# valerio98-lab/DQL_multirotor_landing

Measured on AMD Instinct MI355X. Metric: env-steps/sec (whole node), higher is better.
Workload: dtype f32

## Files before the change

dql_multirotor_landing_amd/csrc/dql_device.hpp:

```cpp
#pragma once
#define DQL_ASM_PIN(...) asm volatile("" : __VA_ARGS__)
#define DQL_ASM_BLOCK(text) asm volatile(text ::: "memory")
#define DQL_ASM_VMOV(dst, src) asm("v_mov_b32 %0, %1" : "=v"(dst) : "s"(src))
#define DQL_ASM_FMA_LIT(d, x, k, y) asm("v_fmamk_f32 %0, %1, %2, %3" : "=v"(d) : "v"(x), "n"(__builtin_bit_cast(int, k)), "v"(y))
#define DQL_ASM_FMA_V(d, x, k, y) asm("v_fma_f32 %0, %1, %2, %3" : "=v"(d) : "v"(x), "v"(k), "v"(y))
#define DQL_ASM_FMA_S(d, x, k, y) asm("v_fma_f32 %0, %1, %2, %3" : "=v"(d) : "v"(x), "s"(k), "v"(y))
#include <hip/hip_runtime.h>
#include <stdint.h>

#include "../../include/dql.h"

#define DQL_DEV __device__ __forceinline__
#ifdef DQL_MARK
#define DQL_SECTION(name) do { __builtin_amdgcn_sched_barrier(0); asm volatile("; SECTION " name ::: "memory"); __builtin_amdgcn_sched_barrier(0); } while (0)
#else
#define DQL_SECTION(name) do { } while (0)
#endif
#ifdef DQL_WAVE_CLOCK
#define DQL_MARK_T(e, k) do { if ((k) == DQL_WAVE_CLOCK) { asm volatile("s_waitcnt vmcnt(0) lgkmcnt(0)" ::: "memory"); (e).mark = wall_clock64(); } } while (0)
#define DQL_WAVE_BEGIN(t0) const unsigned long long t0 = wall_clock64()
#define DQL_WAVE_END_VAR(t1) unsigned long long t1 = 0
#define DQL_WAVE_STORED(e, t1) ((t1) = (e).mark)
#define DQL_WAVE_END(t0, t1, elog, n, i, tid) do {                                                                                           \
    if (DQL_WAVE_CLOCK == 7) { asm volatile("s_waitcnt vmcnt(0) lgkmcnt(0)" ::: "memory"); t1 = wall_clock64(); }                            \
// ... 174 lines not shown
    const T t2 = z * fma_(w, T(0.28498786688), T(0.66666662693));
    const T Rr = t2 + t1, hfsq = T(0.5) * f * f, dk = (T)k;
    return dk * T(6.93147180369123816490e-01) - ((hfsq - (s * (hfsq + Rr) + dk * T(1.90821492927058770002e-10))) - f);
  }
  const T t1 = w * (T(3.999999999940941908e-01) + w * (T(2.222219843214978396e-01) + w * T(1.531383769920937332e-01)));
  const T t2 = z * (T(6.666666666666735130e-01) + w * (T(2.857142874366239149e-01) + w * (T(1.818357216161805012e-01) +
               w * T(1.479819860511658591e-01))));
  const T Rr = t2 + t1, hfsq = T(0.5) * f * f, dk = (T)k;
  return dk * T(6.93147180369123816490e-01) - ((hfsq - (s * (hfsq + Rr) + dk * T(1.90821492927058770002e-10))) - f);
}

DQL_DEV void philox4x32(uint32_t c0, uint32_t c1, uint32_t c2, uint32_t c3, uint32_t k0, uint32_t k1, uint32_t out[4], const uint32_t* kv = nullptr) {
#pragma unroll
  for (int r = 0; r < 10; ++r) {
    const uint64_t p0 = (uint64_t)0xD2511F53u * c0, p1 = (uint64_t)0xCD9E8D57u * c2;
    const uint32_t h0 = (uint32_t)(p0 >> 32), l0 = (uint32_t)p0, h1 = (uint32_t)(p1 >> 32), l1 = (uint32_t)p1;
    const uint32_t n0 = h1 ^ c1 ^ (kv ? kv[r] : k0), n2 = h0 ^ c3 ^ (kv ? kv[10 + r] : k1);
    c0 = n0; c1 = l1; c2 = n2; c3 = l0;
    k0 += 0x9E3779B9u; k1 += 0xBB67AE85u;
  }
  out[0] = c0; out[1] = c1; out[2] = c2; out[3] = c3;
}
constexpr uint32_t STREAM_ACTION = 0u, STREAM_INIT = 0xFFFFFFFFu, STREAM_NOISE0 = 16u;
template <typename T> DQL_DEV T u24(uint32_t r) { return (T)(r >> 8) * T(5.9604644775390625e-08); }
template <typename T> DQL_DEV T u24p(uint32_t r) { return (T)((r >> 8) + 1u) * T(5.9604644775390625e-08); }
template <typename T> DQL_DEV void box_muller(uint32_t ra, uint32_t rb, T& n0, T& n1) {
  const T rad = sqrt_(T(-2.0) * det_log(u24p<T>(ra)));
  T s, c;
  det_sincos(T(6.28318530717958623200e+00) * u24<T>(rb), s, c);
  n0 = rad * c; n1 = rad * s;
}

#define DQL_CONST_AS __attribute__((address_space(4)))
template <typename T> struct MdpK {
  T p_max, v_max, a_max, theta_max, delta_theta, beta, sigma_a, min_alt;
  T w_p, w_v, w_theta, w_dur, w_fail, w_succ, delta_t, f_ag, timeout_steps;
  T lim_p[5], lim_v[5], lim_a[5], angles[7];
  T inv_p_max, inv_v_max, inv_a_max, inv_theta_max, dtheta_ratio;
  T tan2_mid[3];
  double gamma;
  int working, goal_logic;
  uint32_t quirks;
};
template <typename T> struct SimK {
  T dt, g, inv_m, I[3], inv_I[3], l, h, kf, km, lkf, kmkf, aup, adn, omax, cd, crd;
  T dtm, dtg, dtI[3];
// ... 539 lines not shown
template <typename T> DQL_DEV void platform_rec_begin(const SimK<T>& s, const Env<T>& e, PlatRec<T>& r) {
  det_sincos(e.mp_phase, r.sn, r.cs);
  platform_step_sincos(s, e, r.sd, r.cd);
}
template <typename T> DQL_DEV void platform_update(const SimK<T>& s, Env<T>& e, PlatRec<T>* rec = nullptr, bool first_in_period = true) {
  if (Fast32<T>::on && rec) {
    if (first_in_period) platform_rec_begin(s, e, *rec);
    platform_set(s, e, rec->sn, rec->cs);
    const T sn = rec->sn, cs = rec->cs;
    const T sd = rec->sd, cd = rec->cd;
    rec->sn = fma_(sn, cd, cs * sd);
    rec->cs = fma_(cs, cd, -(sn * sd));
  } else platform_eval(s, e);
  T ph = fma_(e.mp_w, s.mp_dt, e.mp_phase);
  if (ph >= T(6.28318530717958623200e+00)) ph -= T(6.28318530717958623200e+00);
  e.mp_phase = ph;
}
template <typename T> DQL_DEV void manager_states(const T (&R)[9], T cy, T sy, T vz, T& vz_state, T& yw_state) {
  vz_state = vz;
  const T A00 = fma_(cy, R[0], sy * R[3]), A01 = fma_(cy, R[1], sy * R[4]);
  const T A10 = fma_(cy, R[3], -(sy * R[0])), A11 = fma_(cy, R[4], -(sy * R[1]));
  yw_state = det_atan2(fma_(A10, cy, A11 * sy), fma_(A00, cy, A01 * sy));
}
template <typename T>
DQL_DEV void manager_obs(const SimK<T>& s, Env<T>& e, T cy, T sy, long long mgr_index, uint32_t k0, uint32_t k1,
                         uint32_t step_lo, uint32_t step_hi, uint32_t env_id, uint32_t mgr_in_step, bool with_noise = true, PlatRec<T>* rec = nullptr, const uint32_t* kv = nullptr) {
  const T dxw = e.mp_x - e.p[0], dyw = e.mp_y - e.p[1];
  const T dvx = e.mp_u - e.v[0], dvy = e.mp_v - e.v[1];
  const T rpx = fma_(cy, dxw, sy * dyw), rpy = fma_(cy, dyw, -(sy * dxw));
  const T rvx = fma_(cy, dvx, sy * dvy), rvy = fma_(cy, dvy, -(sy * dvx));
  T opx = rpx, opy = rpy, ovx = rvx, ovy = rvy;
  if (with_noise && s.noisy) {
    uint32_t r[4]; T n0, n1, n2, n3;
    philox4x32(step_lo, step_hi, env_id, STREAM_NOISE0 + mgr_in_step, k0, k1, r, kv);
    box_muller(r[0], r[1], n0, n1); box_muller(r[2], r[3], n2, n3);
    opx = fma_(s.noise_p, n0, opx); opy = fma_(s.noise_p, n1, opy); ovx = fma_(s.noise_v, n2, ovx); ovy = fma_(s.noise_v, n3, ovy);
  }
  T ax_ = T(0.0), ay_ = T(0.0);
  if (!(e.flags & FL_ACC_INIT)) {
    e.vf_x = rvx; if (s.two_axis) e.vf_y = rvy; e.flags |= FL_ACC_INIT;
  } else {
    T dt_;
    if (s.quirks & DQL_Q_FROZEN_ACC_REFERENCE) dt_ = (T)mgr_index * s.mgr_dt;
    else dt_ = s.mgr_dt;
    if (dt_ <= T(0.0)) dt_ = T(0.01);
    if (Fast32<T>::on && !(s.quirks & DQL_Q_FROZEN_ACC_REFERENCE)) {
      ax_ = kalman1d(e.kal_x_x, e.kal_x_P, s.kal_q, s.kal_r, (rvx - e.vf_x) * s.inv_mgr_dt, s.kal_pss, s.kal_kss, s.kal_r_zero != 0);
      if (s.two_axis) ay_ = kalman1d(e.kal_y_x, e.kal_y_P, s.kal_q, s.kal_r, (rvy - e.vf_y) * s.inv_mgr_dt, s.kal_pss, s.kal_kss, s.kal_r_zero != 0);
    } else {
      ax_ = kalman1d(e.kal_x_x, e.kal_x_P, s.kal_q, s.kal_r, (rvx - e.vf_x) / dt_, s.kal_pss, s.kal_kss, s.kal_r_zero != 0);
      if (s.two_axis) ay_ = kalman1d(e.kal_y_x, e.kal_y_P, s.kal_q, s.kal_r, (rvy - e.vf_y) / dt_, s.kal_pss, s.kal_kss, s.kal_r_zero != 0);
    }
    if (!(s.quirks & DQL_Q_FROZEN_ACC_REFERENCE)) { e.vf_x = rvx; if (s.two_axis) e.vf_y = rvy; }
  }
  e.obs_px = opx; e.obs_py = opy; e.obs_vx = ovx; e.obs_vy = ovy; e.obs_ax = ax_; e.obs_ay = ay_;
  if (e.flags & FL_CONTACT) e.flags |= FL_OBS_CONTACT; else e.flags &= ~FL_OBS_CONTACT;
  platform_update(s, e, rec, mgr_in_step == 0);
// ... 200 lines not shown
}

DQL_DEV long long fx_round(double x) {
  x = __builtin_fmin(__builtin_fmax(x, -0x1p50), 0x1p50);
  const double t = x + 0x1.8p52;
  return __double_as_longlong(t) - __double_as_longlong(0x1.8p52);
}

struct StepOut {
  long long target_fx;
  long long target_y_fx;
  long long reward_fx;
  int cell, cell_y;
  int decision, done;
  QRow next;
};

struct PeriodCtx {
  uint32_t k0, k1, step_lo, step_hi;
  int prev_idx, prev_idy, action, action_y;
  bool is_reset;
  bool coin, coin_y;
};
template <typename T, typename TabPtr>
DQL_DEV PeriodCtx period_begin(const SimK<T>& s, Env<T>& e, const QRow& qx, TabPtr qa, TabPtr qb, int mode, uint32_t eps_thr, int ext_action, uint64_t seed,
                               uint32_t env_id, long long step_index, const uint32_t* kv = nullptr) {
  PeriodCtx c;
  c.k0 = (uint32_t)seed; c.k1 = (uint32_t)(seed >> 32); c.step_lo = (uint32_t)step_index; c.step_hi = (uint32_t)((uint64_t)step_index >> 32);
  uint32_t r[4];
  philox4x32(c.step_lo, c.step_hi, env_id, STREAM_ACTION, c.k0, c.k1, r, kv);
  c.is_reset = (e.flags & FL_DONE) != 0;
  c.prev_idx = e.idx_x; c.prev_idy = e.idx_y;
  const bool two = s.two_axis != 0;
  int action = 2, action_y = 2;
  uint32_t r2[4] = {0u, 0u, 0u, 0u};
  if (two) philox4x32(c.step_lo, c.step_hi, env_id, STREAM_ACTION + 1u, c.k0, c.k1, r2, kv);
  if (c.is_reset) {
    e.step_count = 0; e.cur_check = 0; e.code = DQL_NON_TERMINAL; e.cum_x = T(0.0); e.cum_y = T(0.0);
    e.pitch_sp = T(0.0); e.roll_sp = T(0.0);
    if (!(s.quirks & DQL_Q_SHAPING_SURVIVES_RESET)) { e.shp_p = T(0.0); e.shp_v = T(0.0); e.shp_a = T(0.0); e.shpy_p = T(0.0); e.shpy_v = T(0.0); e.shpy_a = T(0.0); }
    T x0;
    if (s.working == 0 && !s.init_uniform) { T n0, n1; box_muller(r[2], r[3], n0, n1); x0 = s.init_sigma * n0; }
    else x0 = fma_(T(2.0) * u24<T>(r[2]), s.p_max, -s.p_max);
    e.p[0] = place_axis(s.init_uniform, x0, e.mp_x, s.p_max);
    e.p[1] = T(0.0); e.p[2] = s.z_init;
    if (two) {
      T y0;
      if (s.working == 0 && !s.init_uniform) { T n0, n1; box_muller(r2[2], r2[3], n0, n1); y0 = s.init_sigma * n0; }
      else y0 = fma_(T(2.0) * u24<T>(r2[2]), s.p_max, -s.p_max);
      e.p[1] = place_axis(s.init_uniform, y0, e.mp_y, s.p_max);
    }
    e.v[0] = e.v[1] = e.v[2] = T(0.0); e.w[0] = e.w[1] = e.w[2] = T(0.0);
    e.q[0] = T(1.0); e.q[1] = e.q[2] = e.q[3] = T(0.0);
    e.flags &= ~(FL_DONE | FL_CONTACT | FL_OBS_CONTACT);
    e.flags |= FL_WAS_RESET;
  } else {
    e.flags &= ~FL_WAS_RESET;
    if (mode == MODE_EXTERNAL) { action = ext_action & 3; action_y = two ? (ext_action >> 2) & 3 : 2; }
    else {
      const int greedy = agent_predict(qx);
      const bool explore = (mode == MODE_TRAIN) && ((r[0] >> 8) < eps_thr);
      action = explore ? (int)(((uint64_t)r[1] * 3u) >> 32) : greedy;
      if (two) {
        const int greedy_y = agent_predict(qa, qb, c.prev_idy < 0 ? 0 : c.prev_idy);
        const bool explore_y = (mode == MODE_TRAIN) && ((r2[0] >> 8) < eps_thr);
        action_y = explore_y ? (int)(((uint64_t)r2[1] * 3u) >> 32) : greedy_y;
      }
    }
    e.pitch_sp = continuous_action(s, e.pitch_sp, action);
    if (two) e.roll_sp = -continuous_action(s, -e.roll_sp, action_y);
  }
  c.action = action; c.action_y = action_y;
  c.coin = (r[2] >> 31) != 0; c.coin_y = (r2[2] >> 31) != 0;
  e.action = action | (two ? action_y << 2 : 0);
  return c;
}
enum { MDP_VECTOR = 0, MDP_SCALAR = 1, MDP_LITERAL = 2 };
template <typename T, typename M, typename TabPtr>
DQL_DEV StepOut period_end_with(const SimK<T>& s, const M& m, Env<T>& e, const PeriodCtx& c, TabPtr qa, TabPtr qb, int mode);
template <int MDP_SRC, typename T, typename TabPtr>
DQL_DEV StepOut period_end(const SimK<T>& s, const MdpK<T> DQL_CONST_AS* mp, const MdpRun<T>& mr, Env<T>& e, const PeriodCtx& c, TabPtr qa, TabPtr qb, int mode) {
  if constexpr (MDP_SRC == MDP_LITERAL && sizeof(T) == 4) {
    const LitM m{mr.timeout_steps, mr.gamma, s.working, mr.goal_logic, s.quirks};
    return period_end_with(s, m, e, c, qa, qb, mode);
  } else {
    asm volatile("" ::: "memory");
    MdpK<T> m;
    if constexpr (MDP_SRC == MDP_SCALAR) __builtin_memcpy(&m, mp, sizeof(m));
    else m = *(const MdpK<T>*)mp;
    return period_end_with(s, m, e, c, qa, qb, mode);
  }
}
template <typename T, typename M, typename TabPtr>
DQL_DEV StepOut period_end_with(const SimK<T>& s, const M& m, Env<T>& e, const PeriodCtx& c, TabPtr qa, TabPtr qb, int mode) {
  StepOut out; out.cell = -1; out.cell_y = -1; out.decision = 0; out.done = 0; out.target_fx = 0; out.target_y_fx = 0; out.reward_fx = 0;
  const bool two = s.two_axis != 0;
  const int prev_idx = c.prev_idx, prev_idy = c.prev_idy;
  T R[9];
  DQL_SECTION("end_pitch");
  quat_to_R(e.q, R);
  int idx, idy = -1;
  Bins bnx{0, 0, 0}, bny{0, 0, 0};
  if constexpr (Fast32<T>::on) {
    const int bin_x = angle_bin_from_tangent(m, -R[6], fma_(R[0], R[0], R[3] * R[3]), true);
    DQL_SECTION("end_discretise");
    idx = discretise_impl<true>(m, e.obs_px, e.obs_vx, e.obs_ax, T(0.0), bin_x, &bnx);
    if (two) idy = discretise_impl<true>(m, e.obs_py, e.obs_vy, e.obs_ay, T(0.0), angle_bin_from_tangent(m, -R[7], R[8] * R[8], R[8] > T(0.0)), &bny);
  } else {
    const T cyy = sqrt_(fma_(R[0], R[0], R[3] * R[3]));
    const T pitch = det_atan2(-R[6], cyy);
    DQL_SECTION("end_discretise");
    idx = discretise_impl<false>(m, e.obs_px, e.obs_vx, e.obs_ax, pitch, 0, &bnx);
    if (two) { const T roll = det_atan2(R[7], R[8]); idy = discretise_impl<false>(m, e.obs_py, e.obs_vy, e.obs_ay, -roll, 0, &bny); }
  }
  if (idx < 0) { idx = 0; bnx = Bins{0, 0, 0}; }
  e.idx_x = idx;
  if (two) {
    if (idy < 0) { idy = 0; bny = Bins{0, 0, 0}; }
    e.idx_y = idy;
  }
  const int prev_k = e.bin_k, prev_p = e.bin_p, prev_ky = e.bin_ky, prev_py = e.bin_py;
  e.bin_k = bnx.k; e.bin_p = bnx.p; e.bin_ky = bny.k; e.bin_py = bny.p;
  e.reward = T(0.0);
  DQL_SECTION("end_qrow");
  out.next = load_qrow(qa, qb, idx);
  DQL_MARK_T(e, 41);
  if (c.is_reset) return out;
  DQL_SECTION("end_check");
  const bool contact = (e.flags & FL_OBS_CONTACT) != 0;
  e.code = mdp_check(m, e.step_count, e.cur_check, e.code, prev_idx, idx, contact, e.obs_px, e.obs_py, e.p[2], two, prev_idy, idy, &bnx, prev_k, &bny, prev_ky);
  DQL_SECTION("end_reward");
  const T rew = mdp_reward(m, e.shp_p, e.shp_v, e.shp_a, e.cum_x, e.code, idx, e.obs_px, e.obs_vx, e.pitch_sp, &bnx);
  T rew_y = T(0.0);
  if (two) rew_y = mdp_reward(m, e.shpy_p, e.shpy_v, e.shpy_a, e.cum_y, e.code, idy, e.obs_py, e.obs_vy, -e.roll_sp, &bny);
  e.reward = two ? rew + rew_y : rew;
  DQL_MARK_T(e, 42);
  DQL_SECTION("end_target");
  const bool done = e.code <= DQL_TERMINAL_TIMEOUT;
  if (done) e.flags |= FL_DONE;
  out.decision = 1; out.done = done ? 1 : 0;
  out.reward_fx = fx_round((double)rew * (double)(1ll << DQL_TARGET_FRAC_BITS));
  if (two) out.reward_fx += fx_round((double)rew_y * (double)(1ll << DQL_TARGET_FRAC_BITS));
  if (mode == MODE_TRAIN) {
    const bool dbl = !(s.quirks & DQL_Q_UPDATE_TABLE_A_ONLY);
    {
      const bool sel_b = dbl && c.coin;
      const double a0 = out.next.a0, a1 = out.next.a1, a2 = out.next.a2;
      double s0 = a0, s1 = a1, s2 = a2, v0 = a0, v1 = a1, v2 = a2;
      if (dbl) {
// ... 28 lines not shown
      out.cell_y = prev_idy * 3 + c.action_y + (sel_b ? DQL_N_CELLS : 0);
      out.target_y_fx = fx_round(target_y * (double)(1ll << DQL_TARGET_FRAC_BITS));
    }
  }
  return out;
}

template <typename T> struct TickUnroll { static constexpr int n = sizeof(T) == 4 ? 1 : 2; };
constexpr int GROUP = 5;
enum { TICK_PLAIN = 0, TICK_PACKED = 2, TICK_LIT = 3, TICK_PACKED_LITM = 4 };
constexpr bool tick_is_packed(int t) { return t == TICK_PACKED || t == TICK_PACKED_LITM; }
template <int TICK, typename T> struct TickK { static DQL_DEV const SimK<T>& get(const SimK<T>& s) { return s; } };
template <> struct TickK<TICK_PACKED, float> { static DQL_DEV HotK<float> get(const SimK<float>& s) { return make_hot(s); } };
template <> struct TickK<TICK_PACKED_LITM, float> { static DQL_DEV HotK<float> get(const SimK<float>& s) { return make_hot(s); } };
template <> struct TickK<TICK_LIT, float> { static DQL_DEV LitK get(const SimK<float>& s) { return LitK{s.vz_sp, s.yw_sp}; } };
template <int TICK, typename T> struct TickConsts {
  decltype(TickK<TICK, T>::get(*(const SimK<T>*)nullptr)) h;
  PkK pk;
  DQL_DEV explicit TickConsts(const SimK<T>& s) : h(TickK<TICK, T>::get(s)) {
    if constexpr (sizeof(T) == 4 && tick_is_packed(TICK)) pk = make_pkk(h);
  }
};
enum { X_TWO = 0, X_ONLY = 1, X_RUNTIME = 2 };
template <int TICK, int XMODE, bool LEVEL0 = false, typename T, typename TabPtr>
DQL_DEV StepOut agent_period(const SimK<T>& s_in, const TickConsts<TICK, T>& tc, const MdpK<T> DQL_CONST_AS* mp, const MdpRun<T>& mr, Env<T>& e, const QRow& qx, TabPtr qa, TabPtr qb, int mode, uint32_t eps_thr,
                             int ext_action, uint64_t seed, uint32_t env_id, long long step_index, long long mgr0, int sched, const uint32_t* kv = nullptr) {
  SimK<T> s = s_in;
  if constexpr (sizeof(T) == 4 && (TICK == TICK_LIT || TICK == TICK_PLAIN)) {
    if constexpr (LEVEL0) DQL_ASM_PIN("+s"(s.quirks), "+s"(s.init_uniform), "+s"(mode));
    else DQL_ASM_PIN("+s"(s.quirks), "+s"(s.working), "+s"(s.init_uniform), "+s"(mode));
  }
  if constexpr (LEVEL0) s.working = 0;
  DQL_SECTION("period_begin");
  const PeriodCtx c = period_begin(s, e, qx, qa, qb, mode, eps_thr, ext_action, seed, env_id, step_index, kv);
  T B[9];
  DQL_SECTION("make_B");
  make_B(e.pitch_sp, e.roll_sp, B);
  DQL_SECTION("tick_setup");
  constexpr bool HOT = tick_is_packed(TICK);
  const auto& h = tc.h;
  T yw_lo = T(h.yw_lo), yw_hi = T(h.yw_hi), yw_wind = T(h.yw_wind), c375 = T(0.375), low_z = T(h.low_z);
  if constexpr (sizeof(T) == 4 && TICK == TICK_LIT) {
    DQL_ASM_PIN("+s"(yw_wind), "+s"(yw_hi), "+s"(c375));
    DQL_ASM_PIN("+s"(low_z));
    if (T(h.yw_lo) == -T(h.yw_hi)) yw_lo = -yw_hi;
  }
  DQL_MARK_T(e, 3);
  DQL_PHASE(e, 1);
  T R[9], cy, sy, ct = T(1.0), rn = T(1.0);
  uint32_t mgr_in_step = 0;
  PlatRec<T> prec;
  prec = PlatRec<T>{};
  const int n_ticks = sched & 0xff;
  int phase = (sched >> 8) & 0xff;
  long long mgr_index = mgr0;
  const uint32_t last_mgr = (uint32_t)(sched >> 16);
  auto manager_tick = [&]() {
    DQL_SECTION("manager");
    DQL_PHASE(e, 2);
    manager_states(R, cy, sy, e.v[2], e.vz_state, e.yw_state);
    manager_obs(s, e, cy, sy, mgr_index, c.k0, c.k1, c.step_lo, c.step_hi, env_id, mgr_in_step, mgr_in_step == last_mgr, &prec, kv);
    ++mgr_in_step; ++mgr_index;
    DQL_PHASE(e, 3);
  };
  auto control_and_plant = [&]() {
    DQL_SECTION("pid");
    const T thrust = pid_output(h, h.vz_kp, h.vz_ki, h.vz_lo, h.vz_hi, h.vz_wind, h.vz_sp, e.vz_state, e.vz_i, e.vz_x1, e.vz_x2, e.vz_y1, e.vz_y2, e.vz_y3);
    const T r_cmd = pid_output(h, h.yw_kp, h.yw_ki, yw_lo, yw_hi, yw_wind, h.yw_sp, e.yw_state, e.yw_i, e.yw_x1, e.yw_x2, e.yw_y1, e.yw_y2, e.yw_y3);
    T cmd[4];
    DQL_SECTION("attitude");
    attitude(h, R, e.w, B, cy, sy, ct, rn, r_cmd, thrust, cmd, XMODE == X_ONLY || (XMODE == X_RUNTIME && s.two_axis == 0));
    DQL_SECTION("motor_body");
    plant_step(h, e, R);
    rotor_filter<true>(h, e, cmd);
    DQL_SECTION("platform_contact");
    platform_contact(h, e, low_z);
  };
  if constexpr (sizeof(T) == 4 && tick_is_packed(TICK)) {
    TickPk ts;
    pack_tick(e, ts);
    const PkK& pk = tc.pk;
    const f2 B01 = f2{B[0], B[1]}, B34 = f2{B[3], B[4]}, B67 = f2{B[6], B[7]};
    const float B2 = B[2], B5 = B[5], B8 = B[8];
    RotPk rp;
    auto tick_pk = [&](bool mgr) {
      DQL_SECTION("rot");
      rot_pk(ts, rp);
      if (mgr) {
        e.p[0] = opq(ts.p01.x); e.p[1] = opq(ts.p01.y); e.p[2] = ts.p2; e.v[0] = opq(ts.v01.x); e.v[1] = opq(ts.v01.y); e.v[2] = ts.v2;
        e.mp_x = opq(ts.mp_xy.x); e.mp_y = opq(ts.mp_xy.y); e.mp_u = opq(ts.mp_uv.x); e.mp_v = opq(ts.mp_uv.y);
        {
          DQL_SECTION("manager");
          DQL_PHASE(e, 2);
          float Rm[9];
          rot_to_array(rp, Rm);
          manager_states(Rm, rp.cy, rp.sy, e.v[2], e.vz_state, e.yw_state);
          manager_obs(s, e, rp.cy, rp.sy, mgr_index, c.k0, c.k1, c.step_lo, c.step_hi, env_id, mgr_in_step, mgr_in_step == last_mgr, &prec, kv);
          ++mgr_in_step; ++mgr_index;
          DQL_PHASE(e, 3);
        }
        ts.pid_state = mk2(e.vz_state, e.yw_state); ts.mp_xy = mk2(e.mp_x, e.mp_y); ts.mp_uv = mk2(e.mp_u, e.mp_v);
      }
      DQL_SECTION("tick_pk");
      if constexpr (XMODE == X_RUNTIME) {
        if (s.two_axis == 0) physics_tick_pk<true>(h, pk, ts, rp, B01, B34, B67, B2, B5, B8, e.flags);
        else physics_tick_pk<false>(h, pk, ts, rp, B01, B34, B67, B2, B5, B8, e.flags);
      } else physics_tick_pk<XMODE == X_ONLY>(h, pk, ts, rp, B01, B34, B67, B2, B5, B8, e.flags);
    };
    int left = n_ticks;
    for (;;) {
      while (left > 0 && !(s.div == GROUP && phase == 0 && left >= GROUP)) {
        tick_pk(phase == 0);
        phase = (phase + 1 == s.div) ? 0 : phase + 1;
        --left;
      }
      if (left == 0) break;
      do {
        tick_pk(true);
#pragma unroll
        for (int k = 1; k < GROUP; ++k) tick_pk(false);
        left -= GROUP;
      } while (left >= GROUP);
    }
    unpack_tick(ts, e);
  } else {
    int togo = phase == 0 ? 0 : s.div - phase;
#pragma unroll TickUnroll<T>::n
    for (int i = 0; i < n_ticks; ++i) {
      if constexpr (sizeof(T) == 8) asm volatile("" ::: "memory");
      DQL_SECTION("rot");
      quat_to_R(e.q, R); yaw_cs(R, cy, sy, ct, rn, c375);
      if (togo == 0) { manager_tick(); togo = s.div; }
      --togo;
      control_and_plant();
    }
  }
  DQL_SECTION("epilogue");
  DQL_MARK_T(e, 4);
  DQL_PHASE(e, 2);
  const StepOut o = period_end<(TICK == TICK_LIT || TICK == TICK_PACKED_LITM) ? MDP_LITERAL : (HOT ? MDP_VECTOR : MDP_SCALAR)>(s, mp, mr, e, c, qa, qb, mode);
  DQL_MARK_T(e, 5);
  DQL_PHASE(e, 4);
  return o;
}

template <typename T> DQL_DEV void load_env(Env<T>& e, const Quad<T>* __restrict__ sr, const int4 iv, long long n, long long i, const SimK<T>& c) {
  const Quad<T> q0 = sr[0 * n + i], q1 = sr[1 * n + i], q2 = sr[2 * n + i], q3 = sr[3 * n + i], q4 = sr[4 * n + i], q5 = sr[5 * n + i];
  const Quad<T> q6 = sr[6 * n + i], q7 = sr[7 * n + i], q8 = sr[8 * n + i], q9 = sr[9 * n + i], q10 = sr[10 * n + i];
  e.p[0] = q0.a; e.p[1] = q0.b; e.p[2] = q0.c; e.v[0] = q0.d;
  e.v[1] = q1.a; e.v[2] = q1.b; e.q[0] = q1.c; e.q[1] = q1.d;
  e.q[2] = q2.a; e.q[3] = q2.b; e.w[0] = q2.c; e.w[1] = q2.d;
  e.w[2] = q3.a; e.om[0] = q3.b; e.om[1] = q3.c; e.om[2] = q3.d;
  e.om[3] = q4.a; e.vz_i = q4.b; e.vz_x1 = q4.c; e.vz_x2 = q4.d;
  e.vz_y1 = q5.a; e.vz_y2 = q5.b; e.vz_y3 = q5.c; e.vz_state = q5.d;
  e.yw_i = q6.a; e.yw_x1 = q6.b; e.yw_x2 = q6.c; e.yw_y1 = q6.d;
  e.yw_y2 = q7.a; e.yw_y3 = q7.b; e.yw_state = q7.c; e.pitch_sp = q7.d;
  e.mp_phase = q8.a; e.mp_x = q8.b; e.mp_u = q8.c; e.vf_x = q8.d;
  e.kal_x_x = q9.a; e.kal_x_P = q9.b; e.shp_p = q9.c; e.shp_v = q9.d;
  e.shp_a = q10.a; e.cum_x = q10.b; e.roll_sp = q10.c; e.mp_y = q10.d;
  if (c.two_axis || c.traj == DQL_TRAJ_EIGHT) {
    const Quad<T> q11 = sr[11 * n + i];
    e.mp_v = q11.a; e.vf_y = q11.b; e.kal_y_x = q11.c; e.kal_y_P = q11.d;
  } else { e.mp_v = T(0.0); e.vf_y = T(0.0); e.kal_y_x = T(0.0); e.kal_y_P = T(1.0); }
// ... 31 lines not shown
```

dql_multirotor_landing_amd/csrc/dql_hip.hip:

```cpp
#include <hip/hip_runtime.h>
#include <limits>
#include <rccl/rccl.h>

#include <dlfcn.h>
#include <unistd.h>

#include <cmath>
#include <cstddef>
#include <cstdio>
#include <cstdlib>
#include <cstring>
#include <string>
#include <type_traits>
#include <vector>

#include "dql_device.hpp"
#include "dql_host_consts.hpp"
#include "dql_rollout.hpp"
#include "dql_learner.hpp"
#include "dql_team.hpp"
#include "dql_advance.hpp"
#include "dql_recipes.hpp"
#include "dql_score.hpp"
#include "dql_score_map.hpp"
// ... 221 lines not shown
  const double* qa; const double* qb; unsigned long long* acc_cur;
  double* qa_m; double* qb_m; double* cnt_m; double* qa_pub; double* qb_pub; long long* acc_prev; long long* window;
  StatsDev* stats;
  const char DQL_CONST_AS* mdp;
  unsigned long long* elog;
  unsigned long long* faults;
  FoldK fold;
  long long step_index;
  unsigned long long seed;
  long long mgr0[DQL_MAX_PERIODS];
  int sched[DQL_MAX_PERIODS];
  unsigned int eps_thr; int have_prev, working, pad_;
};
template <typename T> struct PopArgs {
  StepArgs<T> s;
  const PopAgentDesc DQL_CONST_AS* desc;
  int blocks_per_agent, writer_blocks, n_active, pad_;
  int agent[DQL_MAX_AGENTS];
};

constexpr int step_waves_per_simd(int block) { return block == 512 ? 4 : 2; }
constexpr int step_min_waves_per_simd(int block, int real_size) { return block >= 512 ? step_waves_per_simd(block) : (real_size == 8 && block == 256 ? 2 : 1); }
template <typename T> DQL_DEV SimK<T> x_only(SimK<T> c) { c.two_axis = 0; return c; }
template <typename T> struct TickLds { char unused; };
template <> struct TickLds<double> { SimK<double> k; };
struct AnyLevel {};
template <typename T, int BLOCK, int TICK, int XMODE, typename... LEVEL> __global__ __launch_bounds__(BLOCK) __attribute__((amdgpu_waves_per_eu(step_min_waves_per_simd(BLOCK, (int)sizeof(T)), step_waves_per_simd(BLOCK)))) void k_step(StepArgs<T> a) {
  constexpr bool LEVEL0 = sizeof...(LEVEL) == 0;
  static_assert(!LEVEL0 || (sizeof(T) == 4 && (TICK == TICK_LIT || TICK == TICK_PACKED_LITM) && XMODE == X_ONLY), "level-0 instances exist for the x-axis literal-MDP layouts only");
  constexpr bool STAGED = BLOCK > 64;
  __shared__ unsigned long long sT[STAGED ? 2 * DQL_N_CELLS : 1];
  __shared__ unsigned int sM[STAGED ? 2 * DQL_N_CELLS : 1];
  __shared__ unsigned long long sStat[4 + 7];
  DQL_PHASE_BEGIN(clk_start);
  warm_kernarg<(int)sizeof(StepArgs<T>)>();
  const int tid = threadIdx.x;
  DQL_WAVE_BEGIN(clk0);
  if ((int)blockIdx.x >= a.env_blocks) {
    const int c = ((int)blockIdx.x - a.env_blocks) * BLOCK + tid;
    if (c < DQL_N_CELLS) {
      double qa = a.qa_m[c], qb = a.qb_m[c];
      if (a.have_prev) {
        qa = fold_cell(a.fold, a.qa_m, a.cnt_m, a.acc_prev, a.window, a.windowed, c);
        qb = fold_cell(a.fold, a.qb_m, a.cnt_m, a.acc_prev + DQL_ACC_B, a.window + DQL_ACC_B, a.windowed, c);
      }
      a.qa_pub[c] = qa; a.qb_pub[c] = qb;
// ... 2 lines not shown
  }
  const int ncell = (a.c.working + 1) * DQL_CELLS_PER_LEVEL;
  const int n_tab = (a.c.quirks & DQL_Q_UPDATE_TABLE_A_ONLY) ? 1 : 2;
  const long long i = (long long)blockIdx.x * BLOCK + tid;
  long long dec = 0, don = 0, rfx = 0;
  bool goal = false;
  Env<T> e;
  QRow qx = QRow{0.0, 0.0, 0.0, 0.0, 0.0, 0.0};
  if (i < a.n) {
    const int4 iv = a.si[i];
    qx = load_qrow(a.qa, a.qb, (unsigned)iv.x < (unsigned)(DQL_N_CELLS / DQL_N_ACTIONS) ? iv.x : 0);
    load_env(e, a.sr, iv, a.n, i, XMODE == X_ONLY ? x_only(a.c) : a.c);
  }
  SimK<T> cfgk = a.c;
  if constexpr (XMODE == X_ONLY) cfgk.two_axis = 0;
  if constexpr (sizeof(T) == 4 && BLOCK < 512) cfgk = period_consts_in_vgprs(cfgk);
  uint32_t kv_[20];
  const uint32_t* kv = nullptr;
  if constexpr (sizeof(T) == 4 && BLOCK < 512 && (TICK == TICK_LIT || TICK == TICK_PLAIN)) {
#pragma unroll
    for (int r = 0; r < 10; ++r) { kv_[r] = to_vgpr((uint32_t)a.seed + (uint32_t)r * 0x9E3779B9u); kv_[10 + r] = to_vgpr((uint32_t)(a.seed >> 32) + (uint32_t)r * 0xBB67AE85u); }
    kv = kv_;
  }
  if (STAGED) {
    for (int t = 0; t < n_tab; ++t)
      for (int c = tid; c < ncell; c += BLOCK) { sT[t * DQL_N_CELLS + c] = 0ull; sM[t * DQL_N_CELLS + c] = 0u; }
    if (tid < 4 + 7) sStat[tid] = 0ull;
    __syncthreads();
  }
  DQL_WAVE_END_VAR(clk1);
  if (i < a.n) {
    DQL_MARK_T(e, 2);
    DQL_PHASE_LOADED(e, clk_start);
  }
  long long dec_w = 0, don_w = 0, rfx_w = 0;
  long long rfx_lane = 0;
  unsigned code_w[7] = {0u, 0u, 0u, 0u, 0u, 0u, 0u};
  __shared__ TickLds<T> sTickK;
  if constexpr (sizeof(T) == 8) {
    if (tid == 0) sTickK.k = cfgk;
    __syncthreads();
  }
  const TickConsts<TICK, T> tc([&]() -> const SimK<T>& { if constexpr (sizeof(T) == 8) return sTickK.k; else return cfgk; }());
  constexpr bool FAIR = (TICK == TICK_PLAIN || TICK == TICK_LIT) && BLOCK >= 128;
  unsigned prio_role = 0u;
  bool fair_prio = false;
  if constexpr (FAIR) {
    fair_prio = a.fair_prio != 0;
    if (fair_prio) {
      unsigned hw_id;
      asm volatile("s_getreg_b32 %0, hwreg(HW_REG_HW_ID)" : "=s"(hw_id));
      prio_role = hw_id & 1u;
    }
  }
  for (int p = 0; p < a.n_periods; ++p) {
    if (fair_prio) { if ((((unsigned)p) ^ prio_role) & 1u) asm volatile("s_setprio 1"); else asm volatile("s_setprio 0"); }
    dec = 0; don = 0; rfx = 0; goal = false;
    int done_code = -1;
    if (i < a.n) {
      const int ext = (a.mode == MODE_EXTERNAL) ? (int)a.actions[i] : 2;
      if (a.mode == MODE_EXTERNAL) {
        const int ax = ext & 3, ay = (ext >> 2) & 3;
        if (ax > 2 || ay > 2 || (ext >> 4) || (!a.c.two_axis && ay != 0 && ay != 2)) atomicAdd(&a.stats->bad_actions, 1ull);
      }
      const StepOut o = agent_period<TICK, XMODE, LEVEL0>(cfgk, tc, a.mdp, a.mdp_run, e, qx, a.qa, a.qb, a.mode, a.eps_thr, ext, a.seed, (uint32_t)(a.env_id_offset + i), a.step_index + p, a.mgr0[p], a.sched[p], kv);
      DQL_SECTION("accumulate");
      if (STAGED) {
        if (o.cell >= 0) { atomicAdd(&sT[o.cell], (unsigned long long)o.target_fx); atomicAdd(&sM[o.cell], 1u); }
        if (o.cell_y >= 0) { atomicAdd(&sT[o.cell_y], (unsigned long long)o.target_y_fx); atomicAdd(&sM[o.cell_y], 1u); }
      } else {
        if (o.cell >= 0) { const int g = o.cell + (o.cell >= DQL_N_CELLS ? DQL_N_CELLS : 0); atomicAdd(&a.acc_cur[g], (unsigned long long)o.target_fx); atomicAdd(&a.acc_cur[DQL_N_CELLS + g], 1ull); }
        if (o.cell_y >= 0) { const int g = o.cell_y + (o.cell_y >= DQL_N_CELLS ? DQL_N_CELLS : 0); atomicAdd(&a.acc_cur[g], (unsigned long long)o.target_y_fx); atomicAdd(&a.acc_cur[DQL_N_CELLS + g], 1ull); }
      }
      qx = o.next;
      dec = o.decision; don = o.done; rfx = o.reward_fx;
      if (o.done) { done_code = e.code; goal = e.code == DQL_TERMINAL_SUCCESS; }
    }
    if (ELOG_MASKS && a.elog) {
      const unsigned long long dm = __ballot(don != 0), sm = __ballot(goal);
      const long long w = i >> 6, nw = (a.n + 63) >> 6;
      unsigned long long* row = a.elog + (size_t)p * 2 * (size_t)nw;
      if ((tid & 63) == 0 && w < nw) { row[w] = dm; row[nw + w] = sm; }
    }
    dec_w += __popcll(__ballot(dec != 0)); don_w += __popcll(__ballot(don != 0)); rfx_lane += rfx;
    if (i < a.n) DQL_PHASE(e, 5);
    if (__ballot(done_code >= 0)) {
#pragma unroll
      for (int k = 0; k <= DQL_TERMINAL_TIMEOUT; ++k) code_w[k] += (unsigned)__popcll(__ballot(done_code == k));
// ... 79 lines not shown
    load_env(e, a.sr, iv, a.n, i, XMODE == X_ONLY ? x_only(a.c) : a.c);
    DQL_MARK_T(e, 2);
    DQL_PHASE_LOADED(e, clk_start);
  }
  long long dec_w = 0, don_w = 0, rfx_w = 0;
  long long rfx_lane = 0;
  unsigned code_w[7] = {0u, 0u, 0u, 0u, 0u, 0u, 0u};
  SimK<T> cfgk = a.c;
  if constexpr (XMODE == X_ONLY) cfgk.two_axis = 0;
  if constexpr (sizeof(T) == 4 && BLOCK < 512) cfgk = period_consts_in_vgprs(cfgk);
  __shared__ TickLds<T> sTickK;
  if constexpr (sizeof(T) == 8) {
    if (tid == 0) sTickK.k = cfgk;
    __syncthreads();
  }
  const TickConsts<TICK, T> tc([&]() -> const SimK<T>& { if constexpr (sizeof(T) == 8) return sTickK.k; else return cfgk; }());
  uint32_t kv_[20];
  const uint32_t* kv = nullptr;
  if constexpr (sizeof(T) == 4 && BLOCK < 512 && (TICK == TICK_LIT || TICK == TICK_PLAIN)) {
#pragma unroll
    for (int r = 0; r < 10; ++r) { kv_[r] = to_vgpr((uint32_t)a.seed + (uint32_t)r * 0x9E3779B9u); kv_[10 + r] = to_vgpr((uint32_t)(a.seed >> 32) + (uint32_t)r * 0xBB67AE85u); }
    kv = kv_;
  }
  constexpr bool FAIR = (TICK == TICK_PLAIN || TICK == TICK_LIT) && BLOCK >= 128;
  unsigned prio_role = 0u;
  bool fair_prio = false;
  if constexpr (FAIR) {
    fair_prio = a.fair_prio != 0;
    if (fair_prio) {
      unsigned hw_id;
      asm volatile("s_getreg_b32 %0, hwreg(HW_REG_HW_ID)" : "=s"(hw_id));
      prio_role = hw_id & 1u;
    }
  }
  for (int p = 0; p < a.n_periods; ++p) {
    if (fair_prio) { if ((((unsigned)p) ^ prio_role) & 1u) asm volatile("s_setprio 1"); else asm volatile("s_setprio 0"); }
    dec = 0; don = 0; rfx = 0; goal = false;
    int done_code = -1;
    if (i < a.n) {
      const int ext = (a.mode == MODE_EXTERNAL) ? (int)a.actions[i] : 2;
      if (a.mode == MODE_EXTERNAL) {
        const int ax = ext & 3, ay = (ext >> 2) & 3;
        if (ax > 2 || ay > 2 || (ext >> 4) || (!a.c.two_axis && ay != 0 && ay != 2)) atomicAdd(&a.stats->bad_actions, 1ull);
      }
      const StepOut o = agent_period<TICK, XMODE>(cfgk, tc, a.mdp, a.mdp_run, e, qx, a.qa, a.qb, a.mode, a.eps_thr, ext, a.seed, (uint32_t)(a.env_id_offset + i), a.step_index + p, d->mgr0[p], d->sched[p], kv);
      DQL_SECTION("accumulate");
      const bool okx = (unsigned)o.cell < 2u * DQL_N_CELLS, oky = (unsigned)o.cell_y < 2u * DQL_N_CELLS;
      if ((o.cell >= 0 && !okx) || (o.cell_y >= 0 && !oky)) atomicAdd(d->faults, (unsigned long long)((o.cell >= 0 && !okx) + (o.cell_y >= 0 && !oky)));
      if (STAGED) {
        if (okx) { atomicAdd(&sT[o.cell], (unsigned long long)o.target_fx); atomicAdd(&sM[o.cell], 1u); }
        if (oky) { atomicAdd(&sT[o.cell_y], (unsigned long long)o.target_y_fx); atomicAdd(&sM[o.cell_y], 1u); }
      } else {
        if (okx) { const int g = o.cell + (o.cell >= DQL_N_CELLS ? DQL_N_CELLS : 0); atomicAdd(&a.acc_cur[g], (unsigned long long)o.target_fx); atomicAdd(&a.acc_cur[DQL_N_CELLS + g], 1ull); }
        if (oky) { const int g = o.cell_y + (o.cell_y >= DQL_N_CELLS ? DQL_N_CELLS : 0); atomicAdd(&a.acc_cur[g], (unsigned long long)o.target_y_fx); atomicAdd(&a.acc_cur[DQL_N_CELLS + g], 1ull); }
      }
      qx = o.next;
      dec = o.decision; don = o.done; rfx = o.reward_fx;
      if (o.done) { done_code = e.code; goal = e.code == DQL_TERMINAL_SUCCESS; }
    }
    if (ELOG_MASKS && a.elog) {
      const unsigned long long dm = __ballot(don != 0), sm = __ballot(goal);
      const long long w = i >> 6, nw = (a.n + 63) >> 6;
      unsigned long long* row = a.elog + (size_t)p * 2 * (size_t)nw;
      if ((tid & 63) == 0 && w < nw) { row[w] = dm; row[nw + w] = sm; }
    }
    dec_w += __popcll(__ballot(dec != 0)); don_w += __popcll(__ballot(don != 0)); rfx_lane += rfx;
    if (i < a.n) DQL_PHASE(e, 5);
    if (__ballot(done_code >= 0)) {
// ... 1323 lines not shown
```

Baseline: 7.838 billion.

## Precompute Philox front rounds and draw next period's action randoms ahead

Splits Philox into a per-launch env-dependent part, a per-step uniform part and per-lane partial rounds, so that the first two rounds are shared across the action and noise streams of a step. The action random numbers for the next period are drawn at the end of the current period, after the Q-row load is issued, so the integer work can hide that load's latency. In exchange the pipe state must stay live in registers across the whole period, which raises VGPR pressure and may hurt occupancy. The path is enabled only for f32 with blocks smaller than 512 and the LIT/PLAIN tick variants.

After: 7.909 billion (median of 6 runs). No clear change (+0.9%).

```diff
diff --git a/dql_multirotor_landing_amd/csrc/dql_device.hpp b/dql_multirotor_landing_amd/csrc/dql_device.hpp
--- a/dql_multirotor_landing_amd/csrc/dql_device.hpp
+++ b/dql_multirotor_landing_amd/csrc/dql_device.hpp
@@ -220,6 +220,67 @@
   out[0] = c0; out[1] = c1; out[2] = c2; out[3] = c3;
 }
 constexpr uint32_t STREAM_ACTION = 0u, STREAM_INIT = 0xFFFFFFFFu, STREAM_NOISE0 = 16u;
+struct PhiloxFront {
+  uint32_t env_hi, env_lo;
+  uint32_t k0, k1, step_hi, u_hi, u_lo;
+  uint32_t c3, p1_hi, p1_lo;
+};
+DQL_DEV void philox_front_launch(PhiloxFront& f, uint32_t env_id) {
+  const uint64_t p = (uint64_t)0xCD9E8D57u * env_id;
+  f.env_hi = (uint32_t)(p >> 32); f.env_lo = (uint32_t)p;
+}
+DQL_DEV void philox_front_uniform(PhiloxFront& f, uint32_t step_lo, uint32_t step_hi, uint32_t k0, uint32_t k1) {
+  const uint64_t u = (uint64_t)0xD2511F53u * step_lo;
+  f.k0 = k0; f.k1 = k1; f.step_hi = step_hi; f.u_hi = (uint32_t)(u >> 32); f.u_lo = (uint32_t)u;
+}
+DQL_DEV void philox_front_lanes(PhiloxFront& f) {
+  const uint32_t c0 = f.env_hi ^ f.step_hi ^ f.k0;
+  const uint64_t p0 = (uint64_t)0xD2511F53u * c0;
+  const uint32_t c2 = (uint32_t)(p0 >> 32) ^ f.u_lo ^ (f.k1 + 0xBB67AE85u);
+  const uint64_t p1 = (uint64_t)0xCD9E8D57u * c2;
+  f.c3 = (uint32_t)p0; f.p1_hi = (uint32_t)(p1 >> 32); f.p1_lo = (uint32_t)p1;
+}
+DQL_DEV uint64_t philox_front_stream(const PhiloxFront& f, uint32_t stream) { return (uint64_t)0xCD9E8D57u * (f.u_hi ^ stream ^ f.k1); }
+DQL_DEV void philox_draw_with(const PhiloxFront& f, uint64_t q, uint32_t out[4], const uint32_t* kv = nullptr) {
+  uint32_t c0 = ((uint32_t)(q >> 32) ^ (f.k0 + 0x9E3779B9u)) ^ f.env_lo, c1 = (uint32_t)q, c2, c3;
+  {
+    const uint64_t p0 = (uint64_t)0xD2511F53u * c0;
+    c0 = f.p1_hi ^ c1 ^ (kv ? kv[2] : f.k0 + 2u * 0x9E3779B9u); c1 = f.p1_lo;
+    c2 = (uint32_t)(p0 >> 32) ^ f.c3 ^ (kv ? kv[12] : f.k1 + 2u * 0xBB67AE85u); c3 = (uint32_t)p0;
+  }
+  uint32_t k0 = f.k0 + 3u * 0x9E3779B9u, k1 = f.k1 + 3u * 0xBB67AE85u;
+#pragma unroll
+  for (int r = 3; r < 10; ++r) {
+    const uint64_t p0 = (uint64_t)0xD2511F53u * c0, p1 = (uint64_t)0xCD9E8D57u * c2;
+    const uint32_t h0 = (uint32_t)(p0 >> 32), l0 = (uint32_t)p0, h1 = (uint32_t)(p1 >> 32), l1 = (uint32_t)p1;
+    const uint32_t n0 = h1 ^ c1 ^ (kv ? kv[r] : k0), n2 = h0 ^ c3 ^ (kv ? kv[10 + r] : k1);
+    c0 = n0; c1 = l1; c2 = n2; c3 = l0;
+    k0 += 0x9E3779B9u; k1 += 0xBB67AE85u;
+  }
+  out[0] = c0; out[1] = c1; out[2] = c2; out[3] = c3;
+}
+DQL_DEV void philox_draw(const PhiloxFront& f, uint32_t stream, uint32_t out[4], const uint32_t* kv = nullptr) { philox_draw_with(f, philox_front_stream(f, stream), out, kv); }
+struct PhiloxPipe {
+  PhiloxFront f;
+  uint32_t r[4], r2[4];
+  uint64_t seed;
+  long long step_next;
+  const uint32_t* kv;
+  bool more;
+};
+DQL_DEV void philox_pipe_period(PhiloxPipe& pp, bool two) {
+  philox_front_uniform(pp.f, (uint32_t)pp.step_next, (uint32_t)((uint64_t)pp.step_next >> 32), (uint32_t)pp.seed, (uint32_t)(pp.seed >> 32));
+  philox_front_lanes(pp.f);
+  philox_draw(pp.f, STREAM_ACTION, pp.r, pp.kv);
+  if (two) philox_draw(pp.f, STREAM_ACTION + 1u, pp.r2, pp.kv);
+  pp.step_next = (long long)((uint64_t)pp.step_next + 1u);
+}
+DQL_DEV void philox_pipe_launch(PhiloxPipe& pp, uint32_t env_id, uint64_t seed, long long step_index, bool two, const uint32_t* kv) {
+  pp.seed = seed; pp.step_next = step_index; pp.kv = kv; pp.more = false;
+  pp.r2[0] = pp.r2[1] = pp.r2[2] = pp.r2[3] = 0u;
+  philox_front_launch(pp.f, env_id);
+  philox_pipe_period(pp, two);
+}
 template <typename T> DQL_DEV T u24(uint32_t r) { return (T)(r >> 8) * T(5.9604644775390625e-08); }
 template <typename T> DQL_DEV T u24p(uint32_t r) { return (T)((r >> 8) + 1u) * T(5.9604644775390625e-08); }
 template <typename T> DQL_DEV void box_muller(uint32_t ra, uint32_t rb, T& n0, T& n1) {
@@ -805,9 +866,10 @@
   const T A10 = fma_(cy, R[3], -(sy * R[0])), A11 = fma_(cy, R[4], -(sy * R[1]));
   yw_state = det_atan2(fma_(A10, cy, A11 * sy), fma_(A00, cy, A01 * sy));
 }
-template <typename T>
+template <bool FRONT = false, typename T>
 DQL_DEV void manager_obs(const SimK<T>& s, Env<T>& e, T cy, T sy, long long mgr_index, uint32_t k0, uint32_t k1,
-                         uint32_t step_lo, uint32_t step_hi, uint32_t env_id, uint32_t mgr_in_step, bool with_noise = true, PlatRec<T>* rec = nullptr, const uint32_t* kv = nullptr) {
+                         uint32_t step_lo, uint32_t step_hi, uint32_t env_id, uint32_t mgr_in_step, bool with_noise = true, PlatRec<T>* rec = nullptr, const uint32_t* kv = nullptr,
+                         const PhiloxFront* front = nullptr) {
   const T dxw = e.mp_x - e.p[0], dyw = e.mp_y - e.p[1];
   const T dvx = e.mp_u - e.v[0], dvy = e.mp_v - e.v[1];
   const T rpx = fma_(cy, dxw, sy * dyw), rpy = fma_(cy, dyw, -(sy * dxw));
@@ -815,7 +877,8 @@
   T opx = rpx, opy = rpy, ovx = rvx, ovy = rvy;
   if (with_noise && s.noisy) {
     uint32_t r[4]; T n0, n1, n2, n3;
-    philox4x32(step_lo, step_hi, env_id, STREAM_NOISE0 + mgr_in_step, k0, k1, r, kv);
+    if constexpr (FRONT) philox_draw(*front, STREAM_NOISE0 + mgr_in_step, r, kv);
+    else philox4x32(step_lo, step_hi, env_id, STREAM_NOISE0 + mgr_in_step, k0, k1, r, kv);
     box_muller(r[0], r[1], n0, n1); box_muller(r[2], r[3], n2, n3);
     opx = fma_(s.noise_p, n0, opx); opy = fma_(s.noise_p, n1, opy); ovx = fma_(s.noise_v, n2, ovx); ovy = fma_(s.noise_v, n3, ovy);
   }
@@ -1062,19 +1125,23 @@
   bool is_reset;
   bool coin, coin_y;
 };
-template <typename T, typename TabPtr>
+template <bool PIPE = false, typename T, typename TabPtr>
 DQL_DEV PeriodCtx period_begin(const SimK<T>& s, Env<T>& e, const QRow& qx, TabPtr qa, TabPtr qb, int mode, uint32_t eps_thr, int ext_action, uint64_t seed,
-                               uint32_t env_id, long long step_index, const uint32_t* kv = nullptr) {
+                               uint32_t env_id, long long step_index, const uint32_t* kv = nullptr, PhiloxPipe* pipe = nullptr) {
   PeriodCtx c;
   c.k0 = (uint32_t)seed; c.k1 = (uint32_t)(seed >> 32); c.step_lo = (uint32_t)step_index; c.step_hi = (uint32_t)((uint64_t)step_index >> 32);
   uint32_t r[4];
-  philox4x32(c.step_lo, c.step_hi, env_id, STREAM_ACTION, c.k0, c.k1, r, kv);
+  if constexpr (PIPE) { r[0] = pipe->r[0]; r[1] = pipe->r[1]; r[2] = pipe->r[2]; r[3] = pipe->r[3]; }
+  else philox4x32(c.step_lo, c.step_hi, env_id, STREAM_ACTION, c.k0, c.k1, r, kv);
   c.is_reset = (e.flags & FL_DONE) != 0;
   c.prev_idx = e.idx_x; c.prev_idy = e.idx_y;
   const bool two = s.two_axis != 0;
   int action = 2, action_y = 2;
   uint32_t r2[4] = {0u, 0u, 0u, 0u};
-  if (two) philox4x32(c.step_lo, c.step_hi, env_id, STREAM_ACTION + 1u, c.k0, c.k1, r2, kv);
+  if (two) {
+    if constexpr (PIPE) { r2[0] = pipe->r2[0]; r2[1] = pipe->r2[1]; r2[2] = pipe->r2[2]; r2[3] = pipe->r2[3]; }
+    else philox4x32(c.step_lo, c.step_hi, env_id, STREAM_ACTION + 1u, c.k0, c.k1, r2, kv);
+  }
   if (c.is_reset) {
     e.step_count = 0; e.cur_check = 0; e.code = DQL_NON_TERMINAL; e.cum_x = T(0.0); e.cum_y = T(0.0);
     e.pitch_sp = T(0.0); e.roll_sp = T(0.0);
@@ -1116,23 +1183,23 @@
   return c;
 }
 enum { MDP_VECTOR = 0, MDP_SCALAR = 1, MDP_LITERAL = 2 };
-template <typename T, typename M, typename TabPtr>
-DQL_DEV StepOut period_end_with(const SimK<T>& s, const M& m, Env<T>& e, const PeriodCtx& c, TabPtr qa, TabPtr qb, int mode);
-template <int MDP_SRC, typename T, typename TabPtr>
-DQL_DEV StepOut period_end(const SimK<T>& s, const MdpK<T> DQL_CONST_AS* mp, const MdpRun<T>& mr, Env<T>& e, const PeriodCtx& c, TabPtr qa, TabPtr qb, int mode) {
+template <bool PIPE = false, typename T, typename M, typename TabPtr>
+DQL_DEV StepOut period_end_with(const SimK<T>& s, const M& m, Env<T>& e, const PeriodCtx& c, TabPtr qa, TabPtr qb, int mode, PhiloxPipe* pipe = nullptr);
+template <int MDP_SRC, bool PIPE = false, typename T, typename TabPtr>
+DQL_DEV StepOut period_end(const SimK<T>& s, const MdpK<T> DQL_CONST_AS* mp, const MdpRun<T>& mr, Env<T>& e, const PeriodCtx& c, TabPtr qa, TabPtr qb, int mode, PhiloxPipe* pipe = nullptr) {
   if constexpr (MDP_SRC == MDP_LITERAL && sizeof(T) == 4) {
     const LitM m{mr.timeout_steps, mr.gamma, s.working, mr.goal_logic, s.quirks};
-    return period_end_with(s, m, e, c, qa, qb, mode);
+    return period_end_with<PIPE>(s, m, e, c, qa, qb, mode, pipe);
   } else {
     asm volatile("" ::: "memory");
     MdpK<T> m;
     if constexpr (MDP_SRC == MDP_SCALAR) __builtin_memcpy(&m, mp, sizeof(m));
     else m = *(const MdpK<T>*)mp;
-    return period_end_with(s, m, e, c, qa, qb, mode);
-  }
-}
-template <typename T, typename M, typename TabPtr>
-DQL_DEV StepOut period_end_with(const SimK<T>& s, const M& m, Env<T>& e, const PeriodCtx& c, TabPtr qa, TabPtr qb, int mode) {
+    return period_end_with<PIPE>(s, m, e, c, qa, qb, mode, pipe);
+  }
+}
+template <bool PIPE, typename T, typename M, typename TabPtr>
+DQL_DEV StepOut period_end_with(const SimK<T>& s, const M& m, Env<T>& e, const PeriodCtx& c, TabPtr qa, TabPtr qb, int mode, PhiloxPipe* pipe) {
   StepOut out; out.cell = -1; out.cell_y = -1; out.decision = 0; out.done = 0; out.target_fx = 0; out.target_y_fx = 0; out.reward_fx = 0;
   const bool two = s.two_axis != 0;
   const int prev_idx = c.prev_idx, prev_idy = c.prev_idy;
@@ -1165,6 +1232,12 @@
   DQL_SECTION("end_qrow");
   out.next = load_qrow(qa, qb, idx);
   DQL_MARK_T(e, 41);
+  if constexpr (PIPE) {
+    if (pipe->more) {
+      DQL_SECTION("end_draw");
+      philox_pipe_period(*pipe, two);
+    }
+  }
   if (c.is_reset) return out;
   DQL_SECTION("end_check");
   const bool contact = (e.flags & FL_OBS_CONTACT) != 0;
@@ -1239,9 +1312,9 @@
   }
 };
 enum { X_TWO = 0, X_ONLY = 1, X_RUNTIME = 2 };
-template <int TICK, int XMODE, bool LEVEL0 = false, typename T, typename TabPtr>
+template <int TICK, int XMODE, bool LEVEL0 = false, bool PIPE = false, typename T, typename TabPtr>
 DQL_DEV StepOut agent_period(const SimK<T>& s_in, const TickConsts<TICK, T>& tc, const MdpK<T> DQL_CONST_AS* mp, const MdpRun<T>& mr, Env<T>& e, const QRow& qx, TabPtr qa, TabPtr qb, int mode, uint32_t eps_thr,
-                             int ext_action, uint64_t seed, uint32_t env_id, long long step_index, long long mgr0, int sched, const uint32_t* kv = nullptr) {
+                             int ext_action, uint64_t seed, uint32_t env_id, long long step_index, long long mgr0, int sched, const uint32_t* kv = nullptr, PhiloxPipe* pipe = nullptr) {
   SimK<T> s = s_in;
   if constexpr (sizeof(T) == 4 && (TICK == TICK_LIT || TICK == TICK_PLAIN)) {
     if constexpr (LEVEL0) DQL_ASM_PIN("+s"(s.quirks), "+s"(s.init_uniform), "+s"(mode));
@@ -1249,7 +1322,7 @@
   }
   if constexpr (LEVEL0) s.working = 0;
   DQL_SECTION("period_begin");
-  const PeriodCtx c = period_begin(s, e, qx, qa, qb, mode, eps_thr, ext_action, seed, env_id, step_index, kv);
+  const PeriodCtx c = period_begin<PIPE>(s, e, qx, qa, qb, mode, eps_thr, ext_action, seed, env_id, step_index, kv, pipe);
   T B[9];
   DQL_SECTION("make_B");
   make_B(e.pitch_sp, e.roll_sp, B);
@@ -1276,7 +1349,8 @@
     DQL_SECTION("manager");
     DQL_PHASE(e, 2);
     manager_states(R, cy, sy, e.v[2], e.vz_state, e.yw_state);
-    manager_obs(s, e, cy, sy, mgr_index, c.k0, c.k1, c.step_lo, c.step_hi, env_id, mgr_in_step, mgr_in_step == last_mgr, &prec, kv);
+    if constexpr (PIPE) manager_obs<true>(s, e, cy, sy, mgr_index, c.k0, c.k1, c.step_lo, c.step_hi, env_id, mgr_in_step, mgr_in_step == last_mgr, &prec, kv, &pipe->f);
+    else manager_obs(s, e, cy, sy, mgr_index, c.k0, c.k1, c.step_lo, c.step_hi, env_id, mgr_in_step, mgr_in_step == last_mgr, &prec, kv);
     ++mgr_in_step; ++mgr_index;
     DQL_PHASE(e, 3);
   };
@@ -1312,7 +1386,8 @@
           float Rm[9];
           rot_to_array(rp, Rm);
           manager_states(Rm, rp.cy, rp.sy, e.v[2], e.vz_state, e.yw_state);
-          manager_obs(s, e, rp.cy, rp.sy, mgr_index, c.k0, c.k1, c.step_lo, c.step_hi, env_id, mgr_in_step, mgr_in_step == last_mgr, &prec, kv);
+          if constexpr (PIPE) manager_obs<true>(s, e, rp.cy, rp.sy, mgr_index, c.k0, c.k1, c.step_lo, c.step_hi, env_id, mgr_in_step, mgr_in_step == last_mgr, &prec, kv, &pipe->f);
+          else manager_obs(s, e, rp.cy, rp.sy, mgr_index, c.k0, c.k1, c.step_lo, c.step_hi, env_id, mgr_in_step, mgr_in_step == last_mgr, &prec, kv);
           ++mgr_in_step; ++mgr_index;
           DQL_PHASE(e, 3);
         }
@@ -1355,7 +1430,7 @@
   DQL_SECTION("epilogue");
   DQL_MARK_T(e, 4);
   DQL_PHASE(e, 2);
-  const StepOut o = period_end<(TICK == TICK_LIT || TICK == TICK_PACKED_LITM) ? MDP_LITERAL : (HOT ? MDP_VECTOR : MDP_SCALAR)>(s, mp, mr, e, c, qa, qb, mode);
+  const StepOut o = period_end<(TICK == TICK_LIT || TICK == TICK_PACKED_LITM) ? MDP_LITERAL : (HOT ? MDP_VECTOR : MDP_SCALAR), PIPE>(s, mp, mr, e, c, qa, qb, mode, pipe);
   DQL_MARK_T(e, 5);
   DQL_PHASE(e, 4);
   return o;
diff --git a/dql_multirotor_landing_amd/csrc/dql_hip.hip b/dql_multirotor_landing_amd/csrc/dql_hip.hip
--- a/dql_multirotor_landing_amd/csrc/dql_hip.hip
+++ b/dql_multirotor_landing_amd/csrc/dql_hip.hip
@@ -267,6 +267,9 @@
 constexpr int step_waves_per_simd(int block) { return block == 512 ? 4 : 2; }
 constexpr int step_min_waves_per_simd(int block, int real_size) { return block >= 512 ? step_waves_per_simd(block) : (real_size == 8 && block == 256 ? 2 : 1); }
 template <typename T> DQL_DEV SimK<T> x_only(SimK<T> c) { c.two_axis = 0; return c; }
+constexpr bool step_draws_ahead(int block, int tick, int real_size) { return real_size == 4 && block < 512 && (tick == TICK_LIT || tick == TICK_PLAIN); }
+template <bool PIPE> struct PipeSlot { PhiloxPipe pp; DQL_DEV PhiloxPipe* ptr() { return &pp; } };
+template <> struct PipeSlot<false> { DQL_DEV PhiloxPipe* ptr() { return nullptr; } };
 template <typename T> struct TickLds { char unused; };
 template <> struct TickLds<double> { SimK<double> k; };
 struct AnyLevel {};
@@ -315,6 +318,9 @@
     for (int r = 0; r < 10; ++r) { kv_[r] = to_vgpr((uint32_t)a.seed + (uint32_t)r * 0x9E3779B9u); kv_[10 + r] = to_vgpr((uint32_t)(a.seed >> 32) + (uint32_t)r * 0xBB67AE85u); }
     kv = kv_;
   }
+  constexpr bool PIPE = step_draws_ahead(BLOCK, TICK, (int)sizeof(T));
+  PipeSlot<PIPE> pp;
+  if constexpr (PIPE) philox_pipe_launch(*pp.ptr(), (uint32_t)(a.env_id_offset + i), a.seed, a.step_index, cfgk.two_axis != 0, kv);
   if (STAGED) {
     for (int t = 0; t < n_tab; ++t)
       for (int c = tid; c < ncell; c += BLOCK) { sT[t * DQL_N_CELLS + c] = 0ull; sM[t * DQL_N_CELLS + c] = 0u; }
@@ -351,12 +357,13 @@
     dec = 0; don = 0; rfx = 0; goal = false;
     int done_code = -1;
     if (i < a.n) {
+      if constexpr (PIPE) pp.ptr()->more = p + 1 < a.n_periods;
       const int ext = (a.mode == MODE_EXTERNAL) ? (int)a.actions[i] : 2;
       if (a.mode == MODE_EXTERNAL) {
         const int ax = ext & 3, ay = (ext >> 2) & 3;
         if (ax > 2 || ay > 2 || (ext >> 4) || (!a.c.two_axis && ay != 0 && ay != 2)) atomicAdd(&a.stats->bad_actions, 1ull);
       }
-      const StepOut o = agent_period<TICK, XMODE, LEVEL0>(cfgk, tc, a.mdp, a.mdp_run, e, qx, a.qa, a.qb, a.mode, a.eps_thr, ext, a.seed, (uint32_t)(a.env_id_offset + i), a.step_index + p, a.mgr0[p], a.sched[p], kv);
+      const StepOut o = agent_period<TICK, XMODE, LEVEL0, PIPE>(cfgk, tc, a.mdp, a.mdp_run, e, qx, a.qa, a.qb, a.mode, a.eps_thr, ext, a.seed, (uint32_t)(a.env_id_offset + i), a.step_index + p, a.mgr0[p], a.sched[p], kv, pp.ptr());
       DQL_SECTION("accumulate");
       if (STAGED) {
         if (o.cell >= 0) { atomicAdd(&sT[o.cell], (unsigned long long)o.target_fx); atomicAdd(&sM[o.cell], 1u); }
@@ -482,6 +489,9 @@
     for (int r = 0; r < 10; ++r) { kv_[r] = to_vgpr((uint32_t)a.seed + (uint32_t)r * 0x9E3779B9u); kv_[10 + r] = to_vgpr((uint32_t)(a.seed >> 32) + (uint32_t)r * 0xBB67AE85u); }
     kv = kv_;
   }
+  constexpr bool PIPE = step_draws_ahead(BLOCK, TICK, (int)sizeof(T));
+  PipeSlot<PIPE> pp;
+  if constexpr (PIPE) philox_pipe_launch(*pp.ptr(), (uint32_t)(a.env_id_offset + i), a.seed, a.step_index, cfgk.two_axis != 0, kv);
   constexpr bool FAIR = (TICK == TICK_PLAIN || TICK == TICK_LIT) && BLOCK >= 128;
   unsigned prio_role = 0u;
   bool fair_prio = false;
@@ -498,12 +508,13 @@
     dec = 0; don = 0; rfx = 0; goal = false;
     int done_code = -1;
     if (i < a.n) {
+      if constexpr (PIPE) pp.ptr()->more = p + 1 < a.n_periods;
       const int ext = (a.mode == MODE_EXTERNAL) ? (int)a.actions[i] : 2;
       if (a.mode == MODE_EXTERNAL) {
         const int ax = ext & 3, ay = (ext >> 2) & 3;
         if (ax > 2 || ay > 2 || (ext >> 4) || (!a.c.two_axis && ay != 0 && ay != 2)) atomicAdd(&a.stats->bad_actions, 1ull);
       }
-      const StepOut o = agent_period<TICK, XMODE>(cfgk, tc, a.mdp, a.mdp_run, e, qx, a.qa, a.qb, a.mode, a.eps_thr, ext, a.seed, (uint32_t)(a.env_id_offset + i), a.step_index + p, d->mgr0[p], d->sched[p], kv);
+      const StepOut o = agent_period<TICK, XMODE, false, PIPE>(cfgk, tc, a.mdp, a.mdp_run, e, qx, a.qa, a.qb, a.mode, a.eps_thr, ext, a.seed, (uint32_t)(a.env_id_offset + i), a.step_index + p, d->mgr0[p], d->sched[p], kv, pp.ptr());
       DQL_SECTION("accumulate");
       const bool okx = (unsigned)o.cell < 2u * DQL_N_CELLS, oky = (unsigned)o.cell_y < 2u * DQL_N_CELLS;
       if ((o.cell >= 0 && !okx) || (o.cell_y >= 0 && !oky)) atomicAdd(d->faults, (unsigned long long)((o.cell >= 0 && !okx) + (o.cell_y >= 0 && !oky)));
```
